# BinomialLLC/basis_universal

Measured on AMD Instinct MI355X. Metric: encoder Mpixels/s (ETC1S frontend hot path), higher is better.
Workload: dtype u8/int32; 1 GPU; 4096x4096 synthetic RGBA (SURVEY 8d recipe, seed 1234), ETC1S -q128 comp_level 1, basisu_frontend init+compress with tiles resident in HBM; blocks=1048576, max_endpoint_clusters=2416, max_selector_clusters=2731, final_endpoint_clusters=2413, final_selector_clusters=2277, images_in_flight_per_gpu=1, parallelism=1 x one image per GPU (no collective)

## Files before the change

### basis_universal_amd/csrc/etc1s_device.h

```cpp
#pragma once
#include <hip/hip_runtime.h>
#include <stdint.h>

namespace bu {

__device__ __constant__ static const int k_inten_a[8] = {2, 5, 9, 13, 18, 24, 33, 47};
__device__ __constant__ static const int k_inten_b[8] = {8, 17, 29, 42, 60, 80, 106, 183};

__device__ __forceinline__ int inten_delta(int table, int sel) {
    const int v = (sel == 0 || sel == 3) ? k_inten_b[table] : k_inten_a[table];
    return (sel < 2) ? -v : v;
}

__device__ __forceinline__ int clamp255(int v) { return min(max(v, 0), 255); }
__device__ __forceinline__ int scale5(int c) { return (c << 3) | (c >> 2); }

struct cvec { int x, y, z; };

template <bool PERCEPTUAL>
__device__ __forceinline__ cvec to_cvec(int r, int g, int b) {
    cvec c;
    if (PERCEPTUAL) {
        const int l = r * 14 + g * 45 + b * 5;
        c.x = l; c.y = r * 64 - l; c.z = b * 64 - l;
    } else {
        c.x = r; c.y = g; c.z = b;
    }
    return c;
}

template <bool PERCEPTUAL>
__device__ __forceinline__ uint32_t cdist(const cvec& a, const cvec& b) {
    const int dx = a.x - b.x, dy = a.y - b.y, dz = a.z - b.z;
    if (PERCEPTUAL) {
        const uint32_t l2 = (uint32_t)__mul24(dx, dx) >> 5;
        const uint32_t cr = (uint32_t)__mul24(dy, dy) >> 5;
        const uint32_t cb = (uint32_t)__mul24(dz, dz) >> 5;
        const uint32_t cr26 = (cr << 4) + (cr << 3) + (cr << 1);
        const uint32_t cb3 = (cb << 1) + cb;
        return l2 + (cr26 >> 7) + (cb3 >> 7);
    } else {
        return (uint32_t)(__mul24(dx, dx) + __mul24(dy, dy) + __mul24(dz, dz));
    }
}

__device__ __forceinline__ bool base_unclamped(int br, int bg, int bb, int table) {
    const int b = k_inten_b[table];
    return min(br, min(bg, bb)) - b >= 0 && max(br, max(bg, bb)) + b <= 255;
}
__device__ __forceinline__ uint32_t chroma_term(int dy, int dz) {
    const uint32_t cr = (uint32_t)__mul24(dy, dy) >> 5;
    const uint32_t cb = (uint32_t)__mul24(dz, dz) >> 5;
    const uint32_t cr26 = (cr << 4) + (cr << 3) + (cr << 1);
    const uint32_t cb3 = (cb << 1) + cb;
    return (cr26 >> 7) + (cb3 >> 7);
}
struct chroma_moments { int my, mz, r1y, r1z, r2y, r2z; };
__device__ __forceinline__ uint32_t chroma_lower_bound(const chroma_moments& t, int cy, int cz) {
    const int ey = t.my - cy, ez = t.mz - cz;
    const int A = (int)((uint32_t)__mul24(ey, ey) >> 6) + t.r2y + (__mul24(ey, t.r1y) >> 9);
    const int B = (int)((uint32_t)__mul24(ez, ez) >> 6) + t.r2z + (__mul24(ez, t.r1z) >> 9);
    return (uint32_t)max(((__mul24(A, 26) + __mul24(B, 3)) >> 2) - 36, 0);
}
__device__ __forceinline__ uint32_t min_luma_term(int dx0, int a64, int b64) {
    const int m = dx0 < 0 ? -dx0 : dx0;
    const int ea = m - a64, eb = m - b64;
    return min((uint32_t)__mul24(ea, ea), (uint32_t)__mul24(eb, eb)) >> 5;
}

struct mixed_min { uint32_t luma_sq, full; };
__device__ __forceinline__ uint32_t mixed_min_total(const mixed_min& m, uint32_t chroma) { return min((m.luma_sq >> 5) + chroma, m.full); }
template <bool PERCEPTUAL>
__device__ __forceinline__ void block_cvecs(cvec out[4], int br, int bg, int bb, int table) {
    const int a = k_inten_a[table], b = k_inten_b[table];
    out[0] = to_cvec<PERCEPTUAL>(clamp255(br - b), clamp255(bg - b), clamp255(bb - b));
    out[1] = to_cvec<PERCEPTUAL>(clamp255(br - a), clamp255(bg - a), clamp255(bb - a));
    out[2] = to_cvec<PERCEPTUAL>(clamp255(br + a), clamp255(bg + a), clamp255(bb + a));
    out[3] = to_cvec<PERCEPTUAL>(clamp255(br + b), clamp255(bg + b), clamp255(bb + b));
}

__device__ __forceinline__ cvec select_cvec(const cvec bc[4], uint32_t s) {
    const int x0 = bc[0].x, x1 = bc[1].x, x2 = bc[2].x, x3 = bc[3].x, y0 = bc[0].y, y1 = bc[1].y, y2 = bc[2].y, y3 = bc[3].y;
    const int z0 = bc[0].z, z1 = bc[1].z, z2 = bc[2].z, z3 = bc[3].z;
    const bool odd = (s & 1u) != 0, up = (s & 2u) != 0;
    cvec c;
    c.x = up ? (odd ? x3 : x2) : (odd ? x1 : x0);
    c.y = up ? (odd ? y3 : y2) : (odd ? y1 : y0);
    c.z = up ? (odd ? z3 : z2) : (odd ? z1 : z0);
    return c;
}

template <bool PERCEPTUAL>
__device__ __forceinline__ uint32_t min_err4(const cvec& p, const cvec bc[4]) {
    const uint32_t e0 = cdist<PERCEPTUAL>(p, bc[0]), e1 = cdist<PERCEPTUAL>(p, bc[1]);
    const uint32_t e2 = cdist<PERCEPTUAL>(p, bc[2]), e3 = cdist<PERCEPTUAL>(p, bc[3]);
    return min(min(e0, e1), min(e2, e3));
}

template <bool PERCEPTUAL>
__device__ __forceinline__ uint32_t best_sel4(const cvec& p, const cvec bc[4]) {
    uint32_t be = cdist<PERCEPTUAL>(p, bc[0]), bs = 0;
#pragma unroll
    for (uint32_t s = 1; s < 4; s++) {
        const uint32_t e = cdist<PERCEPTUAL>(p, bc[s]);
        if (e < be) { be = e; bs = s; }
    }
    return bs;
}

__device__ __forceinline__ cvec pixel_cvec_lin(uint32_t rgba) {
    cvec c; c.x = rgba & 255; c.y = (rgba >> 8) & 255; c.z = (rgba >> 16) & 255; return c;
}
template <bool PERCEPTUAL>
__device__ __forceinline__ cvec pixel_cvec(uint32_t rgba) {
    return to_cvec<PERCEPTUAL>(rgba & 255, (rgba >> 8) & 255, (rgba >> 16) & 255);
}

__device__ __forceinline__ uint32_t hash_hsieh3(uint32_t r, uint32_t g, uint32_t b) {
    uint32_t h = 3u;
    h += r | (g << 8);
    h ^= h << 16;
    h ^= ((uint32_t)(int32_t)(int8_t)b) << 18;
    h += h >> 11;
    h ^= h << 3;  h += h >> 5;
    h ^= h << 4;  h += h >> 17;
    h ^= h << 25; h += h >> 6;
    return h;
}

__device__ __forceinline__ uint64_t etc1s_header_bits(uint32_t r5, uint32_t g5, uint32_t b5, uint32_t inten) {
    return ((uint64_t)r5 << 59) | ((uint64_t)g5 << 51) | ((uint64_t)b5 << 43) | ((uint64_t)inten << 37) | ((uint64_t)inten << 34) |
           (1ull << 33) | (1ull << 32);
}
__device__ __forceinline__ uint32_t selector_bits(uint32_t x, uint32_t y, uint32_t sel) {
    const uint32_t raw = (0x4Bu >> (sel * 2)) & 3u;
    const uint32_t bit = x * 4 + y;
    return ((raw & 1u) << bit) | ((raw >> 1) << (16 + bit));
}
__device__ __forceinline__ uint64_t bswap64(uint64_t v) { return __builtin_bswap64(v); }

__device__ __forceinline__ void unpack_etc1s_header(uint64_t mem_le, uint32_t& r5, uint32_t& g5, uint32_t& b5, uint32_t& inten) {
    const uint64_t v = bswap64(mem_le);
    r5 = (uint32_t)(v >> 59) & 31; g5 = (uint32_t)(v >> 51) & 31; b5 = (uint32_t)(v >> 43) & 31; inten = (uint32_t)(v >> 37) & 7;
}
__device__ __forceinline__ uint32_t selector_from_bits(uint32_t lo32, uint32_t x, uint32_t y) {
    const uint32_t bit = x * 4 + y;
    const uint32_t raw = ((lo32 >> bit) & 1u) | (((lo32 >> (16 + bit)) & 1u) << 1);
    return (0x1Eu >> (raw * 2)) & 3u;
}

}
```

### basis_universal_amd/csrc/etc1s_refine_kernels.hip

```cpp
#include <hip/hip_runtime.h>
#include <stdint.h>
#include "etc1s_device.h"
#include "etc1s_kernels.h"
#include "launch_dispatch.h"

namespace bu {


template <bool PERCEPTUAL>
__global__ __launch_bounds__(256) void k_refine_endpoint_clusterization(
    const uint4* __restrict__ pixel_blocks, uint32_t n_blocks, const uint32_t* __restrict__ block_cluster,
    const uint32_t* __restrict__ cluster_params, uint32_t n_clusters, uint32_t n_parents,
    const uint32_t* __restrict__ cand_offsets, const uint32_t* __restrict__ cand_indices, const uint8_t* __restrict__ block_parent,
    uint32_t* __restrict__ out_best) {
    constexpr uint32_t RQ = 256;
    __shared__ uint2 s_q[4][2][RQ];
    __shared__ uint32_t s_qp[4][2][RQ];
    const uint32_t lane = threadIdx.x & 63u;
    const uint32_t block = (uint32_t)__builtin_amdgcn_readfirstlane((int)(blockIdx.x * 4u + (threadIdx.x >> 6)));
    if (block >= n_blocks) return;

    cvec pc[16];
    {
        const uint4* src = pixel_blocks + (size_t)block * 4;
#pragma unroll
        for (int i = 0; i < 4; i++) {
            const uint4 v = src[i];
            pc[i * 4 + 0] = pixel_cvec<PERCEPTUAL>(v.x); pc[i * 4 + 1] = pixel_cvec<PERCEPTUAL>(v.y);
            pc[i * 4 + 2] = pixel_cvec<PERCEPTUAL>(v.z); pc[i * 4 + 3] = pixel_cvec<PERCEPTUAL>(v.w);
        }
    }
    const uint32_t cur = block_cluster[block];
    const uint32_t cur_inten = (cluster_params[cur] >> 24) & 255u;

    uint32_t first = 0, total = n_clusters;
    if (n_parents) {
        const uint32_t p = block_parent[block];
        first = cand_offsets[p];
        total = cand_offsets[p + 1] - first;
    }

    uint64_t best_key = ~0ull;
    uint32_t cur_err = 0xFFFFFFFFu;
    uint2 (*q)[RQ] = s_q[threadIdx.x >> 6];
    uint32_t (*qp)[RQ] = s_qp[threadIdx.x >> 6];
    uint32_t thr;
    {
        const uint32_t prm = cluster_params[cur];
        cvec bc[4];
        block_cvecs<PERCEPTUAL>(bc, scale5((int)(prm & 255u)), scale5((int)((prm >> 8) & 255u)), scale5((int)((prm >> 16) & 255u)), (int)((prm >> 24) & 7u));
        const uint32_t w = reinterpret_cast<const uint32_t*>(pixel_blocks + (size_t)block * 4)[lane & 15u];
        uint32_t e = lane < 16 ? min_err4<PERCEPTUAL>(pixel_cvec<PERCEPTUAL>(w), bc) : 0u;
#pragma unroll
        for (int o = 8; o >= 1; o >>= 1) e += (uint32_t)__shfl_xor((int)e, o, 64);
        thr = (uint32_t)__builtin_amdgcn_readfirstlane((int)e);
    }
    constexpr int FIRST_PX[4] = { 0, 5, 10, 15 };
    constexpr uint64_t REST_PX = 0xEDCB98764321ull;
    const uint32_t* block_words = reinterpret_cast<const uint32_t*>(pixel_blocks + (size_t)block * 4);
    auto sync_queue = [&]() {
        __builtin_amdgcn_fence(__ATOMIC_RELEASE, "wavefront");
        __builtin_amdgcn_wave_barrier();
        __builtin_amdgcn_fence(__ATOMIC_ACQUIRE, "wavefront");
    };
    auto tighten = [&]() {
        uint32_t m = (uint32_t)(best_key >> 32);
#pragma unroll
        for (int o = 32; o >= 1; o >>= 1) m = min(m, (uint32_t)__shfl_xor((int)m, o, 64));
        thr = min(thr, m);
    };
    bool seen_cur = false;
    for (int attempt = 0; attempt < 2; attempt++) {
    for (uint32_t base = 0; base < total; base += RQ) {
        uint32_t n0 = 0, n1 = 0;
#pragma unroll
        for (int i = 0; i < (int)(RQ / 64); i++) {
            const uint32_t k = base + (uint32_t)i * 64u + lane;
            bool take = k < total;
            uint32_t prm = 0, ci = 0;
            if (take) {
                ci = n_parents ? cand_indices[first + k] : k;
                prm = cluster_params[ci];
                take = ((prm >> 24) & 255u) <= cur_inten;
            }
            const bool plain = PERCEPTUAL && base_unclamped(scale5((int)(prm & 255u)), scale5((int)((prm >> 8) & 255u)), scale5((int)((prm >> 16) & 255u)), (int)((prm >> 24) & 7u));
            const uint64_t m0 = __ballot(take && plain), m1 = __ballot(take && !plain);
            const uint32_t r0 = __builtin_amdgcn_mbcnt_hi((uint32_t)(m0 >> 32), __builtin_amdgcn_mbcnt_lo((uint32_t)m0, 0u));
            const uint32_t r1 = __builtin_amdgcn_mbcnt_hi((uint32_t)(m1 >> 32), __builtin_amdgcn_mbcnt_lo((uint32_t)m1, 0u));
            const uint2 e = make_uint2(prm, k | (ci == cur ? 0x80000000u : 0u));
            if (take && plain) q[0][n0 + r0] = e;
            if (take && !plain) q[1][n1 + r1] = e;
            n0 += (uint32_t)__popcll(m0); n1 += (uint32_t)__popcll(m1);
            seen_cur = seen_cur || __ballot(take && ci == cur) != 0ull;
        }
        sync_queue();
        {
            uint32_t ns = 0;
            for (uint32_t j0 = 0; j0 < n0; j0 += 64) {
                const uint32_t j = j0 + lane;
                const bool have = j < n0;
                const uint2 e = q[0][have ? j : 0];
                const int inten = (int)((e.x >> 24) & 7u);
                const cvec bcv = to_cvec<true>(scale5((int)(e.x & 255u)), scale5((int)((e.x >> 8) & 255u)), scale5((int)((e.x >> 16) & 255u)));
                const int a64 = k_inten_a[inten] * 64, b64 = k_inten_b[inten] * 64;
                uint32_t part = 0;
#pragma unroll
                for (int f = 0; f < 4; f++) { const int p = FIRST_PX[f]; part += min_luma_term(pc[p].x - bcv.x, a64, b64) + chroma_term(pc[p].y - bcv.y, pc[p].z - bcv.z); }
                const bool keep = have && part <= thr;
                const uint64_t m = __ballot(keep);
                const uint32_t r = __builtin_amdgcn_mbcnt_hi((uint32_t)(m >> 32), __builtin_amdgcn_mbcnt_lo((uint32_t)m, 0u));
                if (keep) { q[0][ns + r] = e; qp[0][ns + r] = part; }
                ns += (uint32_t)__popcll(m);
            }
            sync_queue();
            for (uint32_t j4 = lane; j4 < ((ns * 4u + 63u) & ~63u); j4 += 64) {
                const uint32_t j = j4 >> 2, part = j4 & 3u;
                const bool have = j < ns;
                const uint2 e = q[0][have ? j : 0];
                const int inten = (int)((e.x >> 24) & 7u);
                const cvec bcv = to_cvec<true>(scale5((int)(e.x & 255u)), scale5((int)((e.x >> 8) & 255u)), scale5((int)((e.x >> 16) & 255u)));
                const int a64 = k_inten_a[inten] * 64, b64 = k_inten_b[inten] * 64;
                uint32_t tot = 0;
#pragma unroll
                for (int i = 0; i < 3; i++) {
                    const cvec p = pixel_cvec<true>(block_words[(REST_PX >> (4u * (part * 3u + (uint32_t)i))) & 15u]);
                    tot += min_luma_term(p.x - bcv.x, a64, b64) + chroma_term(p.y - bcv.y, p.z - bcv.z);
                }
                tot += (uint32_t)__shfl_xor((int)tot, 1, 64);
                tot += (uint32_t)__shfl_xor((int)tot, 2, 64);
                if (have && part == 0) {
                    tot += qp[0][j];
                    best_key = min(best_key, ((uint64_t)tot << 32) | (e.y & 0x7fffffffu));
                    if (e.y >> 31) cur_err = tot;
                }
            }
            if (attempt == 0) tighten();
        }
        {
            uint32_t ns = 0;
            for (uint32_t j0 = 0; j0 < n1; j0 += 64) {
                const uint32_t j = j0 + lane;
                const bool have = j < n1;
                const uint2 e = q[1][have ? j : 0];
                cvec bc[4];
                block_cvecs<PERCEPTUAL>(bc, scale5((int)(e.x & 255u)), scale5((int)((e.x >> 8) & 255u)), scale5((int)((e.x >> 16) & 255u)), (int)((e.x >> 24) & 7u));
                uint32_t part = 0;
#pragma unroll
                for (int f = 0; f < 4; f++) part += min_err4<PERCEPTUAL>(pc[FIRST_PX[f]], bc);
                const bool keep = have && part <= thr;
                const uint64_t m = __ballot(keep);
                const uint32_t r = __builtin_amdgcn_mbcnt_hi((uint32_t)(m >> 32), __builtin_amdgcn_mbcnt_lo((uint32_t)m, 0u));
                if (keep) { q[1][ns + r] = e; qp[1][ns + r] = part; }
                ns += (uint32_t)__popcll(m);
            }
            sync_queue();
            for (uint32_t j4 = lane; j4 < ((ns * 4u + 63u) & ~63u); j4 += 64) {
                const uint32_t j = j4 >> 2, part = j4 & 3u;
                const bool have = j < ns;
                const uint2 e = q[1][have ? j : 0];
                cvec bc[4];
                block_cvecs<PERCEPTUAL>(bc, scale5((int)(e.x & 255u)), scale5((int)((e.x >> 8) & 255u)), scale5((int)((e.x >> 16) & 255u)), (int)((e.x >> 24) & 7u));
                uint32_t tot = 0;
#pragma unroll
                for (int i = 0; i < 3; i++) tot += min_err4<PERCEPTUAL>(pixel_cvec<PERCEPTUAL>(block_words[(REST_PX >> (4u * (part * 3u + (uint32_t)i))) & 15u]), bc);
                tot += (uint32_t)__shfl_xor((int)tot, 1, 64);
                tot += (uint32_t)__shfl_xor((int)tot, 2, 64);
                if (have && part == 0) {
                    tot += qp[1][j];
                    best_key = min(best_key, ((uint64_t)tot << 32) | (e.y & 0x7fffffffu));
                    if (e.y >> 31) cur_err = tot;
                }
            }
            if (attempt == 0) tighten();
        }
        __builtin_amdgcn_wave_barrier();
    }
    if (seen_cur || attempt == 1) break;
    thr = 0xFFFFFFFFu; best_key = ~0ull; cur_err = 0xFFFFFFFFu;
    }
#pragma unroll
    for (int o = 32; o >= 1; o >>= 1) {
        const uint32_t lo = (uint32_t)__shfl_xor((int)(uint32_t)best_key, o, 64);
        const uint32_t hi = (uint32_t)__shfl_xor((int)(uint32_t)(best_key >> 32), o, 64);
        best_key = min(best_key, ((uint64_t)hi << 32) | lo);
        cur_err = min(cur_err, (uint32_t)__shfl_xor((int)cur_err, o, 64));
    }
    if (lane == 0) {
        const uint32_t min_err = (uint32_t)(best_key >> 32);
        const uint32_t k = (uint32_t)best_key;
        uint32_t winner;
        if (best_key == ~0ull) winner = 0;
        else if (min_err != 0 && cur_err == min_err) winner = cur;
        else winner = n_parents ? cand_indices[first + k] : k;
        out_best[block] = winner;
    }
}


constexpr uint32_t RS_SEG = 18;

template <bool PERCEPTUAL>
__global__ __launch_bounds__(256) void k_refine_sort_lists(const uint32_t* __restrict__ cluster_params, uint32_t n_clusters, uint32_t n_parents,
                                                           const uint32_t* __restrict__ cand_offsets, const uint32_t* __restrict__ cand_indices,
                                                           uint2* __restrict__ items, uint32_t* __restrict__ seg) {
    __shared__ uint32_t s_cnt[16], s_pos[16];
    const uint32_t p = blockIdx.x, tid = threadIdx.x;
    uint32_t first = 0, total = n_clusters;
    if (n_parents) { first = cand_offsets[p]; total = cand_offsets[p + 1] - first; }
    if (tid < 16) s_cnt[tid] = 0;
    __syncthreads();
    auto bucket_of = [&](uint32_t prm) -> uint32_t {
        const uint32_t inten = (prm >> 24) & 7u;
        const bool plain = PERCEPTUAL && base_unclamped(scale5((int)(prm & 255u)), scale5((int)((prm >> 8) & 255u)), scale5((int)((prm >> 16) & 255u)), (int)inten);
        return (plain ? 0u : 8u) + inten;
    };
    for (uint32_t k = tid; k < total; k += 256) {
        const uint32_t ci = n_parents ? cand_indices[first + k] : k;
        atomicAdd(&s_cnt[bucket_of(cluster_params[ci])], 1u);
    }
    __syncthreads();
    if (tid == 0) {
        uint32_t run = 0;
        uint32_t* sg = seg + (size_t)p * RS_SEG;
        sg[0] = first;
        for (int b = 0; b < 16; b++) {
            s_pos[b] = run; run += s_cnt[b];
            if (b < 8) sg[2 + b] = run;
            else sg[10 + (b - 8)] = run - sg[9];
            if (b == 7) sg[1] = run;
        }
    }
    __syncthreads();
    for (uint32_t k = tid; k < total; k += 256) {
        const uint32_t ci = n_parents ? cand_indices[first + k] : k;
        const uint32_t prm = cluster_params[ci];
        const uint32_t at = atomicAdd(&s_pos[bucket_of(prm)], 1u);
        items[first + at] = make_uint2(prm, (k << 16) | ci);
    }
}

template <bool PERCEPTUAL>
__global__ __launch_bounds__(256) void k_refine_sorted(const uint4* __restrict__ pixel_blocks, uint32_t n_blocks, const uint32_t* __restrict__ block_cluster,
                                                       const uint32_t* __restrict__ cluster_params, uint32_t n_parents, const uint2* __restrict__ items,
                                                       const uint32_t* __restrict__ seg, const uint8_t* __restrict__ block_parent, uint32_t* __restrict__ out_best) {
    constexpr uint32_t RQ = 256;
    __shared__ uint2 s_q[4][RQ];
    __shared__ uint32_t s_qp[4][RQ];
    const uint32_t lane = threadIdx.x & 63u;
    const uint32_t block = (uint32_t)__builtin_amdgcn_readfirstlane((int)(blockIdx.x * 4u + (threadIdx.x >> 6)));
    if (block >= n_blocks) return;

    cvec pc[16];
    {
        const uint4* src = pixel_blocks + (size_t)block * 4;
#pragma unroll
        for (int i = 0; i < 4; i++) {
            const uint4 v = src[i];
            pc[i * 4 + 0] = pixel_cvec<PERCEPTUAL>(v.x); pc[i * 4 + 1] = pixel_cvec<PERCEPTUAL>(v.y);
            pc[i * 4 + 2] = pixel_cvec<PERCEPTUAL>(v.z); pc[i * 4 + 3] = pixel_cvec<PERCEPTUAL>(v.w);
        }
    }
    chroma_moments cm = { 0, 0, 0, 0, 0, 0 };
    if (PERCEPTUAL) {
        int s1y = 0, s1z = 0;
#pragma unroll
        for (int i = 0; i < 16; i++) { s1y += pc[i].y; s1z += pc[i].z; }
        cm.my = s1y >> 4; cm.mz = s1z >> 4; cm.r1y = s1y - 16 * cm.my; cm.r1z = s1z - 16 * cm.mz;
#pragma unroll
        for (int i = 0; i < 16; i++) {
            const int ry = pc[i].y - cm.my, rz = pc[i].z - cm.mz;
            cm.r2y += (int)((uint32_t)(ry * ry) >> 10); cm.r2z += (int)((uint32_t)(rz * rz) >> 10);
        }
    }
    const uint32_t cur = block_cluster[block];
    const uint32_t cur_prm = cluster_params[cur];
    const uint32_t cur_inten = (cur_prm >> 24) & 7u;
    const uint32_t* sg = seg + (size_t)(n_parents ? block_parent[block] : 0u) * RS_SEG;
    const uint32_t first = sg[0], plain_total = sg[1];
    const uint32_t n_plain = sg[2 + cur_inten], n_clamped = sg[10 + cur_inten];
    const uint2* plain_items = items + first;
    const uint2* clamped_items = items + first + plain_total;

    constexpr uint64_t REST_PX = 0xEDCB98764321ull;
    const uint32_t* block_words = reinterpret_cast<const uint32_t*>(pixel_blocks + (size_t)block * 4);
    uint2* q = s_q[threadIdx.x >> 6];
    uint32_t* qp = s_qp[threadIdx.x >> 6];
    uint64_t best_key = ~0ull;
    uint32_t cur_err = 0xFFFFFFFFu;
    uint32_t thr;
    {
        const int cr = scale5((int)(cur_prm & 255u)), cg = scale5((int)((cur_prm >> 8) & 255u)), cb = scale5((int)((cur_prm >> 16) & 255u));
        uint32_t e = 0;
        if (PERCEPTUAL && base_unclamped(cr, cg, cb, (int)cur_inten)) {
            const cvec bcv = to_cvec<true>(cr, cg, cb);
            const cvec p = pixel_cvec<true>(block_words[lane & 15u]);
            if (lane < 16) e = min_luma_term(p.x - bcv.x, k_inten_a[cur_inten] * 64, k_inten_b[cur_inten] * 64) + chroma_term(p.y - bcv.y, p.z - bcv.z);
        } else {
            cvec bc[4];
            block_cvecs<PERCEPTUAL>(bc, cr, cg, cb, (int)cur_inten);
            if (lane < 16) e = min_err4<PERCEPTUAL>(pixel_cvec<PERCEPTUAL>(block_words[lane & 15u]), bc);
        }
#pragma unroll
        for (int o = 8; o >= 1; o >>= 1) e += (uint32_t)__shfl_xor((int)e, o, 64);
        thr = (uint32_t)__builtin_amdgcn_readfirstlane((int)e);
    }
    auto sync_queue = [&]() {
        __builtin_amdgcn_fence(__ATOMIC_RELEASE, "wavefront");
        __builtin_amdgcn_wave_barrier();
        __builtin_amdgcn_fence(__ATOMIC_ACQUIRE, "wavefront");
    };
    auto tighten = [&]() {
        uint32_t m = (uint32_t)(best_key >> 32);
#pragma unroll
        for (int o = 32; o >= 1; o >>= 1) m = min(m, (uint32_t)__shfl_xor((int)m, o, 64));
        thr = min(thr, m);
    };
    bool seen_cur = false;
    for (int attempt = 0; attempt < 2; attempt++) {
        for (uint32_t base = 0; base < n_plain; base += RQ) {
            const uint32_t n0 = min(RQ, n_plain - base);
            uint32_t ns = 0;
            for (uint32_t j0 = 0; j0 < n0; j0 += 64) {
                const uint32_t j = j0 + lane;
                const bool have = j < n0;
                const uint2 e = plain_items[base + (have ? j : 0)];
                const cvec bcv = to_cvec<true>(scale5((int)(e.x & 255u)), scale5((int)((e.x >> 8) & 255u)), scale5((int)((e.x >> 16) & 255u)));
                const uint32_t part = chroma_lower_bound(cm, bcv.y, bcv.z);
                const bool keep = have && part <= thr;
                const uint64_t m = __ballot(keep);
                const uint32_t r = __builtin_amdgcn_mbcnt_hi((uint32_t)(m >> 32), __builtin_amdgcn_mbcnt_lo((uint32_t)m, 0u));
                if (keep) q[ns + r] = e;
                ns += (uint32_t)__popcll(m);
                seen_cur = seen_cur || __ballot(have && (e.y & 0xffffu) == cur) != 0ull;
            }
            sync_queue();
            for (uint32_t j4 = lane; j4 < ((ns * 4u + 63u) & ~63u); j4 += 64) {
                const uint32_t j = j4 >> 2, part = j4 & 3u;
                const bool have = j < ns;
                const uint2 e = q[have ? j : 0];
                const int inten = (int)((e.x >> 24) & 7u);
                const cvec bcv = to_cvec<true>(scale5((int)(e.x & 255u)), scale5((int)((e.x >> 8) & 255u)), scale5((int)((e.x >> 16) & 255u)));
                const int a64 = k_inten_a[inten] * 64, b64 = k_inten_b[inten] * 64;
                uint32_t tot = 0;
#pragma unroll
                for (int i = 0; i < 4; i++) {
                    const cvec p = pixel_cvec<true>(block_words[part * 4u + (uint32_t)i]);
                    tot += min_luma_term(p.x - bcv.x, a64, b64) + chroma_term(p.y - bcv.y, p.z - bcv.z);
                }
                tot += (uint32_t)__shfl_xor((int)tot, 1, 64);
                tot += (uint32_t)__shfl_xor((int)tot, 2, 64);
                if (have && part == 0) {
                    best_key = min(best_key, ((uint64_t)tot << 32) | e.y);
                    if ((e.y & 0xffffu) == cur) cur_err = tot;
                }
            }
            if (attempt == 0) tighten();
            __builtin_amdgcn_wave_barrier();
        }
        for (uint32_t base = 0; base < n_clamped; base += RQ) {
            const uint32_t n1 = min(RQ, n_clamped - base);
            uint32_t ns = 0;
            for (uint32_t j0 = 0; j0 < n1; j0 += 16) {
                const uint32_t j = j0 + (lane >> 2), f = lane & 3u;
                const bool have = j < n1;
                const uint2 e = clamped_items[base + (have ? j : 0)];
                cvec bc[4];
                block_cvecs<PERCEPTUAL>(bc, scale5((int)(e.x & 255u)), scale5((int)((e.x >> 8) & 255u)), scale5((int)((e.x >> 16) & 255u)), (int)((e.x >> 24) & 7u));
                uint32_t part = min_err4<PERCEPTUAL>(pixel_cvec<PERCEPTUAL>(block_words[f * 5u]), bc);
                part += (uint32_t)__shfl_xor((int)part, 1, 64);
                part += (uint32_t)__shfl_xor((int)part, 2, 64);
                const bool keep = have && f == 0 && part <= thr;
                const uint64_t m = __ballot(keep);
                const uint32_t r = __builtin_amdgcn_mbcnt_hi((uint32_t)(m >> 32), __builtin_amdgcn_mbcnt_lo((uint32_t)m, 0u));
                if (keep) { q[ns + r] = e; qp[ns + r] = part; }
                ns += (uint32_t)__popcll(m);
                seen_cur = seen_cur || __ballot(have && (e.y & 0xffffu) == cur) != 0ull;
            }
            sync_queue();
            for (uint32_t j4 = lane; j4 < ((ns * 4u + 63u) & ~63u); j4 += 64) {
                const uint32_t j = j4 >> 2, part = j4 & 3u;
                const bool have = j < ns;
                const uint2 e = q[have ? j : 0];
                cvec bc[4];
                block_cvecs<PERCEPTUAL>(bc, scale5((int)(e.x & 255u)), scale5((int)((e.x >> 8) & 255u)), scale5((int)((e.x >> 16) & 255u)), (int)((e.x >> 24) & 7u));
                uint32_t tot = 0;
#pragma unroll
                for (int i = 0; i < 3; i++) tot += min_err4<PERCEPTUAL>(pixel_cvec<PERCEPTUAL>(block_words[(REST_PX >> (4u * (part * 3u + (uint32_t)i))) & 15u]), bc);
                tot += (uint32_t)__shfl_xor((int)tot, 1, 64);
                tot += (uint32_t)__shfl_xor((int)tot, 2, 64);
                if (have && part == 0) {
                    tot += qp[j];
                    best_key = min(best_key, ((uint64_t)tot << 32) | e.y);
                    if ((e.y & 0xffffu) == cur) cur_err = tot;
                }
            }
            if (attempt == 0) tighten();
            __builtin_amdgcn_wave_barrier();
        }
        if (seen_cur || attempt == 1) break;
        thr = 0xFFFFFFFFu; best_key = ~0ull; cur_err = 0xFFFFFFFFu;
    }
#pragma unroll
    for (int o = 32; o >= 1; o >>= 1) {
        const uint32_t lo = (uint32_t)__shfl_xor((int)(uint32_t)best_key, o, 64);
        const uint32_t hi = (uint32_t)__shfl_xor((int)(uint32_t)(best_key >> 32), o, 64);
        best_key = min(best_key, ((uint64_t)hi << 32) | lo);
        cur_err = min(cur_err, (uint32_t)__shfl_xor((int)cur_err, o, 64));
    }
    if (lane == 0) {
        const uint32_t min_err = (uint32_t)(best_key >> 32);
        uint32_t winner;
        if (best_key == ~0ull) winner = 0;
        else if (min_err != 0 && cur_err == min_err) winner = cur;
        else winner = (uint32_t)best_key & 0xffffu;
        out_best[block] = winner;
    }
}

static size_t refine_items_bytes(uint32_t n_clusters, size_t lists) { return (lists * n_clusters * sizeof(uint2) + 255) & ~(size_t)255; }

size_t refine_workspace_bytes(uint32_t n_clusters, uint32_t n_parents) {
    if (n_clusters > 65535u) return 0;
    const size_t lists = n_parents ? n_parents : 1;
    return refine_items_bytes(n_clusters, lists) + lists * RS_SEG * sizeof(uint32_t);
}

hipError_t launch_refine_endpoint_clusterization(hipStream_t st, const void* d_pixel_blocks, uint32_t n_blocks, const uint32_t* d_block_cluster,
                                                 const uint8_t* d_cluster_params, uint32_t n_clusters, uint32_t n_parents, const uint32_t* d_cand_offsets,
                                                 const uint32_t* d_cand_indices, const uint8_t* d_block_parent, bool perceptual, uint32_t* d_out_best, void* d_work) {
    if (!n_blocks) return hipSuccess;
    const dim3 grid((n_blocks + 3) / 4), blk(256);
    const uint4* in = static_cast<const uint4*>(d_pixel_blocks);
    const uint32_t* prm = reinterpret_cast<const uint32_t*>(d_cluster_params);
    const bool sorted = d_work && refine_workspace_bytes(n_clusters, n_parents);
    with_bool(perceptual, [&](auto p) {
        constexpr bool P = decltype(p)::value;
        if (sorted) {
            const size_t lists = n_parents ? n_parents : 1;
            uint2* items = static_cast<uint2*>(d_work);
            uint32_t* seg = reinterpret_cast<uint32_t*>(static_cast<char*>(d_work) + refine_items_bytes(n_clusters, lists));
            hipLaunchKernelGGL(k_refine_sort_lists<P>, dim3((uint32_t)lists), blk, 0, st, prm, n_clusters, n_parents, d_cand_offsets, d_cand_indices, items, seg);
            hipLaunchKernelGGL(k_refine_sorted<P>, grid, blk, 0, st, in, n_blocks, d_block_cluster, prm, n_parents, items, seg, d_block_parent, d_out_best);
        } else {
            hipLaunchKernelGGL(k_refine_endpoint_clusterization<P>, grid, blk, 0, st, in, n_blocks, d_block_cluster, prm, n_clusters, n_parents, d_cand_offsets, d_cand_indices,
                               d_block_parent, d_out_best);
        }
    });
    BU_LAUNCH_CHECK();
    return hipSuccess;
}

}
```

Measured before the change: 1239 Mpixels/s.

## Precompute candidate endpoint color vectors in sort pass and stage pixels in LDS

The list-sorting kernel now precomputes, for each candidate, the perceptual base vector and scaled intensity deltas in a widened 16-byte item. For clamped buckets it also writes the four packed block colors to a side buffer. The refine kernel reads these instead of recomputing scale5/to_cvec/block_cvecs per candidate per block. It also converts pixels once into LDS and reworks the clamped full-error pass to one lane per pixel. The costs are more workspace and wider global/LDS loads per candidate, and the partial error is no longer kept in LDS but recomputed over all 16 pixels.

```diff
diff --git a/basis_universal_amd/csrc/etc1s_device.h b/basis_universal_amd/csrc/etc1s_device.h
--- a/basis_universal_amd/csrc/etc1s_device.h
+++ b/basis_universal_amd/csrc/etc1s_device.h
@@ -116,6 +116,11 @@
     return to_cvec<PERCEPTUAL>(rgba & 255, (rgba >> 8) & 255, (rgba >> 16) & 255);
 }
 
+__device__ __forceinline__ uint2 pack_cvec(const cvec& c) { return make_uint2((uint32_t)c.x, ((uint32_t)c.y & 0xffffu) | ((uint32_t)c.z << 16)); }
+__device__ __forceinline__ cvec unpack_cvec(uint32_t x, uint32_t yz) {
+    cvec c; c.x = (int)x; c.y = (int)(yz << 16) >> 16; c.z = (int)yz >> 16; return c;
+}
+
 __device__ __forceinline__ uint32_t hash_hsieh3(uint32_t r, uint32_t g, uint32_t b) {
     uint32_t h = 3u;
     h += r | (g << 8);
diff --git a/basis_universal_amd/csrc/etc1s_refine_kernels.hip b/basis_universal_amd/csrc/etc1s_refine_kernels.hip
--- a/basis_universal_amd/csrc/etc1s_refine_kernels.hip
+++ b/basis_universal_amd/csrc/etc1s_refine_kernels.hip
@@ -202,7 +202,7 @@
 template <bool PERCEPTUAL>
 __global__ __launch_bounds__(256) void k_refine_sort_lists(const uint32_t* __restrict__ cluster_params, uint32_t n_clusters, uint32_t n_parents,
                                                            const uint32_t* __restrict__ cand_offsets, const uint32_t* __restrict__ cand_indices,
-                                                           uint2* __restrict__ items, uint32_t* __restrict__ seg) {
+                                                           uint4* __restrict__ items, uint4* __restrict__ side, uint32_t* __restrict__ seg) {
     __shared__ uint32_t s_cnt[16], s_pos[16];
     const uint32_t p = blockIdx.x, tid = threadIdx.x;
     uint32_t first = 0, total = n_clusters;
@@ -234,18 +234,36 @@
     for (uint32_t k = tid; k < total; k += 256) {
         const uint32_t ci = n_parents ? cand_indices[first + k] : k;
         const uint32_t prm = cluster_params[ci];
-        const uint32_t at = atomicAdd(&s_pos[bucket_of(prm)], 1u);
-        items[first + at] = make_uint2(prm, (k << 16) | ci);
-    }
+        const uint32_t bucket = bucket_of(prm);
+        const uint32_t at = first + atomicAdd(&s_pos[bucket], 1u);
+        const int br = scale5((int)(prm & 255u)), bg = scale5((int)((prm >> 8) & 255u)), bb = scale5((int)((prm >> 16) & 255u)), inten = (int)((prm >> 24) & 7u);
+        const int a = k_inten_a[inten], b = k_inten_b[inten];
+        const uint2 base = pack_cvec(to_cvec<PERCEPTUAL>(br, bg, bb));
+        items[at] = make_uint4((uint32_t)(a * 64) | ((uint32_t)(b * 64) << 16), (k << 16) | ci, base.x, base.y);
+        if (bucket >= 8) {
+            cvec bc[4];
+            block_cvecs<PERCEPTUAL>(bc, br, bg, bb, inten);
+            const uint2 c0 = pack_cvec(bc[0]), c1 = pack_cvec(bc[1]), c2 = pack_cvec(bc[2]), c3 = pack_cvec(bc[3]);
+            side[2 * (size_t)at] = make_uint4(c0.x, c0.y, c1.x, c1.y);
+            side[2 * (size_t)at + 1] = make_uint4(c2.x, c2.y, c3.x, c3.y);
+        }
+    }
+}
+
+template <bool PERCEPTUAL>
+__device__ __forceinline__ uint32_t min_err4_packed(const cvec& p, const uint4& s0, const uint4& s1) {
+    cvec bc[4] = { unpack_cvec(s0.x, s0.y), unpack_cvec(s0.z, s0.w), unpack_cvec(s1.x, s1.y), unpack_cvec(s1.z, s1.w) };
+    return min_err4<PERCEPTUAL>(p, bc);
 }
 
 template <bool PERCEPTUAL>
 __global__ __launch_bounds__(256) void k_refine_sorted(const uint4* __restrict__ pixel_blocks, uint32_t n_blocks, const uint32_t* __restrict__ block_cluster,
-                                                       const uint32_t* __restrict__ cluster_params, uint32_t n_parents, const uint2* __restrict__ items,
-                                                       const uint32_t* __restrict__ seg, const uint8_t* __restrict__ block_parent, uint32_t* __restrict__ out_best) {
+                                                       const uint32_t* __restrict__ cluster_params, uint32_t n_parents, const uint4* __restrict__ items,
+                                                       const uint4* __restrict__ side, const uint32_t* __restrict__ seg, const uint8_t* __restrict__ block_parent,
+                                                       uint32_t* __restrict__ out_best) {
     constexpr uint32_t RQ = 256;
-    __shared__ uint2 s_q[4][RQ];
-    __shared__ uint32_t s_qp[4][RQ];
+    __shared__ uint4 s_q[4][RQ];
+    __shared__ int4 s_px[4][16];
     const uint32_t lane = threadIdx.x & 63u;
     const uint32_t block = (uint32_t)__builtin_amdgcn_readfirstlane((int)(blockIdx.x * 4u + (threadIdx.x >> 6)));
     if (block >= n_blocks) return;
@@ -278,37 +296,38 @@
     const uint32_t* sg = seg + (size_t)(n_parents ? block_parent[block] : 0u) * RS_SEG;
     const uint32_t first = sg[0], plain_total = sg[1];
     const uint32_t n_plain = sg[2 + cur_inten], n_clamped = sg[10 + cur_inten];
-    const uint2* plain_items = items + first;
-    const uint2* clamped_items = items + first + plain_total;
-
-    constexpr uint64_t REST_PX = 0xEDCB98764321ull;
-    const uint32_t* block_words = reinterpret_cast<const uint32_t*>(pixel_blocks + (size_t)block * 4);
-    uint2* q = s_q[threadIdx.x >> 6];
-    uint32_t* qp = s_qp[threadIdx.x >> 6];
+    const uint4* plain_items = items + first;
+    const uint4* clamped_items = items + first + plain_total;
+    const uint4* clamped_side = side + 2 * ((size_t)first + plain_total);
+
+    uint4* q = s_q[threadIdx.x >> 6];
+    int4* px = s_px[threadIdx.x >> 6];
     uint64_t best_key = ~0ull;
     uint32_t cur_err = 0xFFFFFFFFu;
-    uint32_t thr;
-    {
-        const int cr = scale5((int)(cur_prm & 255u)), cg = scale5((int)((cur_prm >> 8) & 255u)), cb = scale5((int)((cur_prm >> 16) & 255u));
-        uint32_t e = 0;
-        if (PERCEPTUAL && base_unclamped(cr, cg, cb, (int)cur_inten)) {
-            const cvec bcv = to_cvec<true>(cr, cg, cb);
-            const cvec p = pixel_cvec<true>(block_words[lane & 15u]);
-            if (lane < 16) e = min_luma_term(p.x - bcv.x, k_inten_a[cur_inten] * 64, k_inten_b[cur_inten] * 64) + chroma_term(p.y - bcv.y, p.z - bcv.z);
-        } else {
-            cvec bc[4];
-            block_cvecs<PERCEPTUAL>(bc, cr, cg, cb, (int)cur_inten);
-            if (lane < 16) e = min_err4<PERCEPTUAL>(pixel_cvec<PERCEPTUAL>(block_words[lane & 15u]), bc);
-        }
-#pragma unroll
-        for (int o = 8; o >= 1; o >>= 1) e += (uint32_t)__shfl_xor((int)e, o, 64);
-        thr = (uint32_t)__builtin_amdgcn_readfirstlane((int)e);
-    }
     auto sync_queue = [&]() {
         __builtin_amdgcn_fence(__ATOMIC_RELEASE, "wavefront");
         __builtin_amdgcn_wave_barrier();
         __builtin_amdgcn_fence(__ATOMIC_ACQUIRE, "wavefront");
     };
+    uint32_t thr;
+    {
+        const cvec p = pixel_cvec<PERCEPTUAL>(reinterpret_cast<const uint32_t*>(pixel_blocks + (size_t)block * 4)[lane & 15u]);
+        if (lane < 16) px[lane] = make_int4(p.x, p.y, p.z, 0);
+        const int cr = scale5((int)(cur_prm & 255u)), cg = scale5((int)((cur_prm >> 8) & 255u)), cb = scale5((int)((cur_prm >> 16) & 255u));
+        uint32_t e = 0;
+        if (PERCEPTUAL && base_unclamped(cr, cg, cb, (int)cur_inten)) {
+            const cvec bcv = to_cvec<true>(cr, cg, cb);
+            if (lane < 16) e = min_luma_term(p.x - bcv.x, k_inten_a[cur_inten] * 64, k_inten_b[cur_inten] * 64) + chroma_term(p.y - bcv.y, p.z - bcv.z);
+        } else {
+            cvec bc[4];
+            block_cvecs<PERCEPTUAL>(bc, cr, cg, cb, (int)cur_inten);
+            if (lane < 16) e = min_err4<PERCEPTUAL>(p, bc);
+        }
+#pragma unroll
+        for (int o = 8; o >= 1; o >>= 1) e += (uint32_t)__shfl_xor((int)e, o, 64);
+        thr = (uint32_t)__builtin_amdgcn_readfirstlane((int)e);
+        sync_queue();
+    }
     auto tighten = [&]() {
         uint32_t m = (uint32_t)(best_key >> 32);
 #pragma unroll
@@ -323,8 +342,8 @@
             for (uint32_t j0 = 0; j0 < n0; j0 += 64) {
                 const uint32_t j = j0 + lane;
                 const bool have = j < n0;
-                const uint2 e = plain_items[base + (have ? j : 0)];
-                const cvec bcv = to_cvec<true>(scale5((int)(e.x & 255u)), scale5((int)((e.x >> 8) & 255u)), scale5((int)((e.x >> 16) & 255u)));
+                const uint4 e = plain_items[base + (have ? j : 0)];
+                const cvec bcv = unpack_cvec(e.z, e.w);
                 const uint32_t part = chroma_lower_bound(cm, bcv.y, bcv.z);
                 const bool keep = have && part <= thr;
                 const uint64_t m = __ballot(keep);
@@ -337,14 +356,13 @@
             for (uint32_t j4 = lane; j4 < ((ns * 4u + 63u) & ~63u); j4 += 64) {
                 const uint32_t j = j4 >> 2, part = j4 & 3u;
                 const bool have = j < ns;
-                const uint2 e = q[have ? j : 0];
-                const int inten = (int)((e.x >> 24) & 7u);
-                const cvec bcv = to_cvec<true>(scale5((int)(e.x & 255u)), scale5((int)((e.x >> 8) & 255u)), scale5((int)((e.x >> 16) & 255u)));
-                const int a64 = k_inten_a[inten] * 64, b64 = k_inten_b[inten] * 64;
+                const uint4 e = q[have ? j : 0];
+                const cvec bcv = unpack_cvec(e.z, e.w);
+                const int a64 = (int)(e.x & 0xffffu), b64 = (int)(e.x >> 16);
                 uint32_t tot = 0;
 #pragma unroll
                 for (int i = 0; i < 4; i++) {
-                    const cvec p = pixel_cvec<true>(block_words[part * 4u + (uint32_t)i]);
+                    const int4 p = px[part * 4u + (uint32_t)i];
                     tot += min_luma_term(p.x - bcv.x, a64, b64) + chroma_term(p.y - bcv.y, p.z - bcv.z);
                 }
                 tot += (uint32_t)__shfl_xor((int)tot, 1, 64);
@@ -363,33 +381,31 @@
             for (uint32_t j0 = 0; j0 < n1; j0 += 16) {
                 const uint32_t j = j0 + (lane >> 2), f = lane & 3u;
                 const bool have = j < n1;
-                const uint2 e = clamped_items[base + (have ? j : 0)];
-                cvec bc[4];
-                block_cvecs<PERCEPTUAL>(bc, scale5((int)(e.x & 255u)), scale5((int)((e.x >> 8) & 255u)), scale5((int)((e.x >> 16) & 255u)), (int)((e.x >> 24) & 7u));
-                uint32_t part = min_err4<PERCEPTUAL>(pixel_cvec<PERCEPTUAL>(block_words[f * 5u]), bc);
+                const uint32_t at = base + (have ? j : 0);
+                const uint4 e = clamped_items[at];
+                const uint4 s0 = clamped_side[2 * (size_t)at], s1 = clamped_side[2 * (size_t)at + 1];
+                const int4 p = px[f * 5u];
+                uint32_t part = min_err4_packed<PERCEPTUAL>(cvec{ p.x, p.y, p.z }, s0, s1);
                 part += (uint32_t)__shfl_xor((int)part, 1, 64);
                 part += (uint32_t)__shfl_xor((int)part, 2, 64);
                 const bool keep = have && f == 0 && part <= thr;
                 const uint64_t m = __ballot(keep);
                 const uint32_t r = __builtin_amdgcn_mbcnt_hi((uint32_t)(m >> 32), __builtin_amdgcn_mbcnt_lo((uint32_t)m, 0u));
-                if (keep) { q[ns + r] = e; qp[ns + r] = part; }
+                if (keep) q[ns + r] = make_uint4(e.x, e.y, at, 0u);
                 ns += (uint32_t)__popcll(m);
                 seen_cur = seen_cur || __ballot(have && (e.y & 0xffffu) == cur) != 0ull;
             }
             sync_queue();
-            for (uint32_t j4 = lane; j4 < ((ns * 4u + 63u) & ~63u); j4 += 64) {
-                const uint32_t j = j4 >> 2, part = j4 & 3u;
+            for (uint32_t j16 = lane; j16 < ((ns * 16u + 63u) & ~63u); j16 += 64) {
+                const uint32_t j = j16 >> 4, pi = j16 & 15u;
                 const bool have = j < ns;
-                const uint2 e = q[have ? j : 0];
-                cvec bc[4];
-                block_cvecs<PERCEPTUAL>(bc, scale5((int)(e.x & 255u)), scale5((int)((e.x >> 8) & 255u)), scale5((int)((e.x >> 16) & 255u)), (int)((e.x >> 24) & 7u));
-                uint32_t tot = 0;
-#pragma unroll
-                for (int i = 0; i < 3; i++) tot += min_err4<PERCEPTUAL>(pixel_cvec<PERCEPTUAL>(block_words[(REST_PX >> (4u * (part * 3u + (uint32_t)i))) & 15u]), bc);
-                tot += (uint32_t)__shfl_xor((int)tot, 1, 64);
-                tot += (uint32_t)__shfl_xor((int)tot, 2, 64);
-                if (have && part == 0) {
-                    tot += qp[j];
+                const uint4 e = q[have ? j : 0];
+                const uint4 s0 = clamped_side[2 * (size_t)e.z], s1 = clamped_side[2 * (size_t)e.z + 1];
+                const int4 p = px[pi];
+                uint32_t tot = min_err4_packed<PERCEPTUAL>(cvec{ p.x, p.y, p.z }, s0, s1);
+#pragma unroll
+                for (int o = 8; o >= 1; o >>= 1) tot += (uint32_t)__shfl_xor((int)tot, o, 64);
+                if (have && pi == 0) {
                     best_key = min(best_key, ((uint64_t)tot << 32) | e.y);
                     if ((e.y & 0xffffu) == cur) cur_err = tot;
                 }
@@ -417,12 +433,14 @@
     }
 }
 
-static size_t refine_items_bytes(uint32_t n_clusters, size_t lists) { return (lists * n_clusters * sizeof(uint2) + 255) & ~(size_t)255; }
+static size_t refine_pad(size_t bytes) { return (bytes + 255) & ~(size_t)255; }
+static size_t refine_items_bytes(uint32_t n_clusters, size_t lists) { return refine_pad(lists * n_clusters * sizeof(uint4)); }
+static size_t refine_side_bytes(uint32_t n_clusters, size_t lists) { return refine_pad(lists * n_clusters * 2 * sizeof(uint4)); }
 
 size_t refine_workspace_bytes(uint32_t n_clusters, uint32_t n_parents) {
     if (n_clusters > 65535u) return 0;
     const size_t lists = n_parents ? n_parents : 1;
-    return refine_items_bytes(n_clusters, lists) + lists * RS_SEG * sizeof(uint32_t);
+    return refine_items_bytes(n_clusters, lists) + refine_side_bytes(n_clusters, lists) + lists * RS_SEG * sizeof(uint32_t);
 }
 
 hipError_t launch_refine_endpoint_clusterization(hipStream_t st, const void* d_pixel_blocks, uint32_t n_blocks, const uint32_t* d_block_cluster,
@@ -437,10 +455,11 @@
         constexpr bool P = decltype(p)::value;
         if (sorted) {
             const size_t lists = n_parents ? n_parents : 1;
-            uint2* items = static_cast<uint2*>(d_work);
-            uint32_t* seg = reinterpret_cast<uint32_t*>(static_cast<char*>(d_work) + refine_items_bytes(n_clusters, lists));
-            hipLaunchKernelGGL(k_refine_sort_lists<P>, dim3((uint32_t)lists), blk, 0, st, prm, n_clusters, n_parents, d_cand_offsets, d_cand_indices, items, seg);
-            hipLaunchKernelGGL(k_refine_sorted<P>, grid, blk, 0, st, in, n_blocks, d_block_cluster, prm, n_parents, items, seg, d_block_parent, d_out_best);
+            uint4* items = static_cast<uint4*>(d_work);
+            uint4* side = reinterpret_cast<uint4*>(static_cast<char*>(d_work) + refine_items_bytes(n_clusters, lists));
+            uint32_t* seg = reinterpret_cast<uint32_t*>(reinterpret_cast<char*>(side) + refine_side_bytes(n_clusters, lists));
+            hipLaunchKernelGGL(k_refine_sort_lists<P>, dim3((uint32_t)lists), blk, 0, st, prm, n_clusters, n_parents, d_cand_offsets, d_cand_indices, items, side, seg);
+            hipLaunchKernelGGL(k_refine_sorted<P>, grid, blk, 0, st, in, n_blocks, d_block_cluster, prm, n_parents, items, side, seg, d_block_parent, d_out_best);
         } else {
             hipLaunchKernelGGL(k_refine_endpoint_clusterization<P>, grid, blk, 0, st, in, n_blocks, d_block_cluster, prm, n_clusters, n_parents, d_cand_offsets, d_cand_indices,
                                d_block_parent, d_out_best);
```

Result: slower. 1198 Mpixels/s (-3.3%).
